# hustvl/OmniMamba

Hardware: AMD Instinct MI355X
Metric: selective-scan M-elements/sec (higher is better)
Workload: dtype bf16

## Files before the change

include/omk.h:

```cpp
#ifndef OMK_H
#define OMK_H
#include <stddef.h>
#include <stdint.h>

#ifdef __cplusplus
extern "C" {
#endif

#define OMK_ABI_VERSION 14
#define OMK_MAX_DIMS 5

typedef enum { OMK_OK = 0, OMK_EINVAL = -1, OMK_EARCH = -2, OMK_ELAUNCH = -3, OMK_EUNSUPPORTED = -4 } omk_status;
typedef enum { OMK_F32 = 0, OMK_BF16 = 1, OMK_F16 = 2, OMK_U8 = 3 , OMK_I32 = 4 ,
               OMK_F8E4M3 = 5  } omk_dtype;
typedef void* omk_stream;

typedef struct {
  void* data;
  int32_t dtype;
  int32_t ndim;
  int64_t shape[OMK_MAX_DIMS];
  int64_t stride[OMK_MAX_DIMS];
} OmkTensor;

int omk_abi_version(void);
const char* omk_last_error(void);
int omk_is_emulated(void);
size_t omk_sizeof(const char* struct_name);

typedef struct {
  OmkTensor x;
  OmkTensor residual;
// ... 55 lines not shown

typedef struct {
  OmkTensor x;
  OmkTensor weight;
  OmkTensor bias;
  OmkTensor initial_states;
  OmkTensor out;
  OmkTensor final_states;
  int32_t silu;
  OmkTensor seq_lens;
} OmkConv1dFwd;
int omk_causal_conv1d_fwd(const OmkConv1dFwd* p, omk_stream stream);

typedef struct {
  OmkTensor x, weight, bias, initial_states;
  OmkTensor dout;
  OmkTensor dx;
  OmkTensor dweight;
  OmkTensor dbias;
  OmkTensor dinitial_states;
  int32_t silu;
  void* workspace;
  size_t workspace_bytes;
} OmkConv1dBwd;
size_t omk_causal_conv1d_bwd_workspace_bytes(const OmkConv1dBwd* p);
int omk_causal_conv1d_bwd(const OmkConv1dBwd* p, omk_stream stream);

typedef struct {
  OmkTensor x;
  OmkTensor conv_state;
  OmkTensor weight, bias;
  OmkTensor out;
  int32_t silu;
  OmkTensor conv_state_indices;
  OmkTensor seq_lens;
} OmkConv1dUpdate;
int omk_causal_conv1d_update(const OmkConv1dUpdate* p, omk_stream stream);

typedef struct {
  OmkTensor state;
  OmkTensor x;
  OmkTensor dt;
  OmkTensor A;
  OmkTensor Bm, Cm;
  OmkTensor D;
  OmkTensor z;
// ... 177 lines not shown
  float top_p, temperature;
  float min_p;
} OmkSample;
int omk_sample(const OmkSample* p, omk_stream stream);

typedef struct {
  OmkTensor logits;
  OmkTensor out_ids;
  const void* top_k;
  const void* top_p;
  const void* temperature;
  const void* min_p;
  const void* seeds;
  const void* steps;
  const void* penalty;
  const void* history;
  const void* history_lens;
  const void* active;
  int64_t history_stride;
  int64_t history_cap;
} OmkSampleRows;
int omk_sample_rows(const OmkSampleRows* p, omk_stream stream);

#ifdef __cplusplus
}
#endif
#endif
```

omnimamba_amd/_capi.py:

```python
from __future__ import annotations

import ctypes as C
from typing import Optional

import torch

OMK_ABI_VERSION = 14
OMK_MAX_DIMS = 5
OMK_EUNSUPPORTED = -4
NL_FORM_GENERIC, NL_FORM_FAST, NL_FORM_BATCHED, NL_FORM_MATRIX = 0, 1, 2, 3
_DT = {torch.float32: 0, torch.bfloat16: 1, torch.float16: 2, torch.uint8: 3, torch.bool: 3, torch.int32: 4,
       torch.float8_e4m3fn: 5}


class OmkTensor(C.Structure):
    _fields_ = [("data", C.c_void_p), ("dtype", C.c_int32), ("ndim", C.c_int32),
                ("shape", C.c_int64 * OMK_MAX_DIMS), ("stride", C.c_int64 * OMK_MAX_DIMS)]


def T(t: Optional[torch.Tensor]) -> OmkTensor:
    o = OmkTensor()
    if t is None:
        return o
    dt = _DT.get(t.dtype)
    if dt is None:
        raise TypeError(f"unsupported dtype {t.dtype} (f32/bf16/f16, u8/bool masks, int32 indices, e4m3 weights only)")
    n = t.dim()
    if n > OMK_MAX_DIMS:
        raise ValueError("too many dims")
    o.data, o.dtype, o.ndim = t.data_ptr(), dt, n
# ... 1 lines not shown
    o.stride[:n] = t.stride()
    return o


def _S(name, fields):
    return type(name, (C.Structure,), {"_fields_": fields})


_t, _f, _i, _i64 = OmkTensor, C.c_float, C.c_int32, C.c_int64
_ws = [("workspace", C.c_void_p), ("workspace_bytes", C.c_size_t)]

AddNormFwd = _S("OmkAddNormFwd", [(n, _t) for n in ("x", "residual", "weight", "bias", "y", "residual_out", "rstd", "mean")]
                + [("eps", _f), ("is_rms_norm", _i)])
AddNormBwd = _S("OmkAddNormBwd", [(n, _t) for n in ("dy", "dresidual_out", "xsum", "weight", "rstd", "mean", "dx",
                                                    "dresidual_in", "dweight", "dbias")] + _ws
                + [("is_rms_norm", _i), ("has_bias", _i)])
NormGatedFwd = _S("OmkNormGatedFwd", [(n, _t) for n in ("x", "z", "weight", "bias", "y", "rstd")]
                  + [("group_size", _i64), ("eps", _f), ("norm_before_gate", _i)])
NormGatedBwd = _S("OmkNormGatedBwd", [(n, _t) for n in ("dy", "x", "z", "weight", "dx", "dz", "dweight")] + _ws
                  + [("group_size", _i64), ("eps", _f), ("norm_before_gate", _i)])
Conv1dFwd = _S("OmkConv1dFwd", [(n, _t) for n in ("x", "weight", "bias", "initial_states", "out", "final_states")]
               + [("silu", _i), ("seq_lens", _t)])
Conv1dBwd = _S("OmkConv1dBwd", [(n, _t) for n in ("x", "weight", "bias", "initial_states", "dout", "dx", "dweight",
                                                  "dbias", "dinitial_states")] + [("silu", _i), ("workspace", C.c_void_p), ("workspace_bytes", C.c_size_t)])
Conv1dUpdate = _S("OmkConv1dUpdate", [(n, _t) for n in ("x", "conv_state", "weight", "bias", "out")] + [("silu", _i), ("conv_state_indices", _t),
                                                                                                        ("seq_lens", _t)])
StateUpdate = _S("OmkStateUpdate", [(n, _t) for n in ("state", "x", "dt", "A", "Bm", "Cm", "D", "z", "dt_bias", "out")]
                 + [("dt_softplus", _i), ("state_batch_indices", _t)])
StateExtend = _S("OmkStateExtend", [(n, _t) for n in ("state", "x", "dt", "A", "Bm", "Cm", "D", "z", "dt_bias", "out")]
                 + [("dt_softplus", _i), ("state_batch_indices", _t), ("seq_lens", _t)])
SelScanFwd = _S("OmkSelScanFwd", [(n, _t) for n in ("u", "delta", "A", "Bm", "Cm", "D", "z", "delta_bias", "out",
                                                    "last_state", "pass_states")] + [("delta_softplus", _i)])
SelScanBwd = _S("OmkSelScanBwd", [(n, _t) for n in ("u", "delta", "A", "Bm", "Cm", "D", "z", "delta_bias", "dout", "du",
                                                    "ddelta", "dA", "dB", "dC", "dD", "dz", "ddelta_bias", "pass_states")] + _ws
                + [("delta_softplus", _i)])
NormLinear = _S("OmkNormLinear", [(n, _t) for n in ("x", "residual", "z", "norm_weight", "weight", "bias", "lora_a", "lora_b",
                                                    "residual_out", "out", "conv_state", "conv_weight", "conv_bias")]
                + [("group_size", C.c_int64), ("conv_offset", C.c_int64), ("eps", _f), ("lora_scale", _f),
                   ("norm_before_gate", _i), ("conv_silu", _i), ("conv_state_indices", _t),
                   ("weight_scale", _t)])
LoraAdd = _S("OmkLoraAdd", [(n, _t) for n in ("out", "h", "lora_b", "mask")] + [("scale", _f)])
LoraUpBwd = _S("OmkLoraUpBwd", [(n, _t) for n in ("dy", "lora_b", "h", "dh", "dlora_b")])
SsdFwd = _S("OmkSsdFwd", [(n, _t) for n in ("x", "dt", "A", "Bm", "Cm", "D", "z", "dt_bias", "initial_states", "out",
                                            "out_x", "final_states", "window_states")] + _ws
            + [("dt_min", _f), ("dt_max", _f), ("dt_softplus", _i), ("chunk_size", _i), ("force_generic", _i), ("flags", _i),
               ("conv_weight", _t), ("conv_bias", _t), ("seq_lens", _t)])
SSD_PRECISE, SSD_KHILO, SSD_EVERY_CHUNK, SSD_NO_SPLIT, SSD_COLUMN_SLICE, SSD_SEQUENTIAL_BWD = 1, 2, 4, 8, 16, 32
SsdBwd = _S("OmkSsdBwd", [(n, _t) for n in ("x", "dt", "A", "Bm", "Cm", "D", "dt_bias", "initial_states", "y", "dout",
                                            "dfinal_states", "dx", "ddt", "dA", "dB", "dC", "dD", "ddt_bias",
                                            "dinitial_states", "window_states")] + _ws
            + [("dt_min", _f), ("dt_max", _f), ("dt_softplus", _i), ("chunk_size", _i), ("force_generic", _i), ("flags", _i)])

CrossEntropy = _S("OmkCrossEntropy", [("logits", _t), ("labels", C.c_void_p), ("losses", _t), ("grad_scale", C.c_void_p),
                                      ("ignore_index", _i64), ("write_grad", _i)])

Sample = _S("OmkSample", [("logits", _t), ("out_ids", _t), ("step_counter", C.c_void_p), ("seed", C.c_uint64), ("offset", C.c_uint64),
                          ("top_k", _i), ("top_p", _f), ("temperature", _f), ("min_p", _f)])
SampleRows = _S("OmkSampleRows", [("logits", _t), ("out_ids", _t)]
                + [(n, C.c_void_p) for n in ("top_k", "top_p", "temperature", "min_p", "seeds", "steps", "penalty", "history", "history_lens", "active")]
                + [("history_stride", _i64), ("history_cap", _i64)])

STRUCTS = {s.__name__: s for s in (Sample, SampleRows, CrossEntropy, OmkTensor, AddNormFwd, AddNormBwd, NormGatedFwd, NormGatedBwd, Conv1dFwd, Conv1dBwd,
                                   Conv1dUpdate, StateUpdate, StateExtend, SelScanFwd, SelScanBwd, NormLinear, LoraAdd, LoraUpBwd, SsdFwd, SsdBwd)}

SYMBOLS = [
    "omk_abi_version", "omk_last_error", "omk_is_emulated", "omk_sizeof", "omk_ssd_last_kernels",
    "omk_add_norm_fwd", "omk_add_norm_bwd_workspace_bytes", "omk_add_norm_bwd",
    "omk_norm_gated_fwd", "omk_norm_gated_bwd_workspace_bytes", "omk_norm_gated_bwd",
    "omk_causal_conv1d_fwd", "omk_causal_conv1d_bwd_workspace_bytes", "omk_causal_conv1d_bwd", "omk_causal_conv1d_update",
    "omk_selective_state_update", "omk_selective_state_extend", "omk_norm_linear", "omk_norm_linear_form", "omk_lora_add", "omk_lora_up_bwd",
    "omk_selective_scan_fwd", "omk_selective_scan_fwd_form", "omk_selective_scan_bwd_form", "omk_selective_scan_bwd_workspace_bytes", "omk_selective_scan_bwd",
    "omk_ssd_scan_fwd_workspace_bytes", "omk_ssd_scan_fwd_window_states_bytes", "omk_ssd_scan_fwd", "omk_ssd_scan_bwd_workspace_bytes", "omk_ssd_scan_bwd",
    "omk_cross_entropy", "omk_lora_up_bwd_parts", "omk_sample", "omk_sample_rows",
]


def bind(lib: C.CDLL) -> C.CDLL:
    lib.omk_abi_version.restype = C.c_int
    lib.omk_last_error.restype = C.c_char_p
    lib.omk_ssd_last_kernels.restype = C.c_char_p
    lib.omk_is_emulated.restype = C.c_int
    lib.omk_sizeof.restype = C.c_size_t
    lib.omk_sizeof.argtypes = [C.c_char_p]
    for s in SYMBOLS:
        fn = getattr(lib, s)
        if s.endswith("_workspace_bytes") or s.endswith("_window_states_bytes"):
            fn.restype = C.c_size_t
            fn.argtypes = [C.c_void_p]
        elif s in ("omk_selective_scan_fwd_form", "omk_selective_scan_bwd_form", "omk_norm_linear_form"):
            fn.restype = C.c_int
            fn.argtypes = [C.c_void_p]
        elif s == "omk_lora_up_bwd_parts":
            fn.restype = C.c_int
            fn.argtypes = [C.c_int64, C.c_int64, C.POINTER(C.c_int32)]
        elif s not in ("omk_abi_version", "omk_last_error", "omk_is_emulated", "omk_sizeof", "omk_ssd_last_kernels"):
            fn.restype = C.c_int
# ... 53 lines not shown
```

omnimamba_amd/csrc/capi.hip:

```cpp
#include "omk_common.h"

namespace omk {
char* err_buf() {
  static thread_local char buf[512] = {0};
  return buf;
}
int fail(int code, const char* fmt, ...) {
  va_list ap;
  va_start(ap, fmt);
  vsnprintf(err_buf(), 512, fmt, ap);
  va_end(ap);
  return code;
}
char* kern_buf() {
  static thread_local char buf[512] = {0};
  return buf;
}
void kernels_reset() { kern_buf()[0] = 0; }
void kernels_note(const char* fmt, ...) {
  char* b = kern_buf();
  size_t n = strlen(b);
  if (n + 2 >= 512) return;
  if (n) b[n++] = ';';
  va_list ap;
// ... 2 lines not shown
  va_end(ap);
}
int finish_launch(const char* what) {
#ifndef OMK_EMU
  hipError_t e = hipGetLastError();
  if (e == hipErrorNoBinaryForGpu || e == hipErrorInvalidDeviceFunction || e == hipErrorSharedObjectInitFailed || e == hipErrorInvalidImage)
    return fail(OMK_EARCH, "%s: no kernel image for this device (%s): libomnimamba_hip is built for gfx950 (MI355X) only", what, hipGetErrorString(e));
  if (e != hipSuccess) return fail(OMK_ELAUNCH, "%s: launch failed: %s", what, hipGetErrorString(e));
#endif
  (void)what;
  return OMK_OK;
}
}

extern "C" {
int omk_abi_version(void) { return OMK_ABI_VERSION; }
const char* omk_last_error(void) { return omk::err_buf(); }
const char* omk_ssd_last_kernels(void) { return omk::kern_buf(); }
size_t omk_sizeof(const char* n) {
#define OMK_SZ(S) if (strcmp(n, #S) == 0) return sizeof(S)
  if (!n) return 0;
  OMK_SZ(OmkTensor); OMK_SZ(OmkAddNormFwd); OMK_SZ(OmkAddNormBwd); OMK_SZ(OmkNormGatedFwd); OMK_SZ(OmkNormGatedBwd);
  OMK_SZ(OmkConv1dFwd); OMK_SZ(OmkConv1dBwd); OMK_SZ(OmkConv1dUpdate); OMK_SZ(OmkStateUpdate); OMK_SZ(OmkStateExtend); OMK_SZ(OmkSelScanFwd);
  OMK_SZ(OmkSelScanBwd); OMK_SZ(OmkNormLinear); OMK_SZ(OmkLoraAdd); OMK_SZ(OmkLoraUpBwd); OMK_SZ(OmkSsdFwd); OMK_SZ(OmkSsdBwd); OMK_SZ(OmkCrossEntropy); OMK_SZ(OmkSample); OMK_SZ(OmkSampleRows);
#undef OMK_SZ
  return 0;
}
int omk_is_emulated(void) {
#ifdef OMK_EMU
  return 1;
#else
  return 0;
#endif
}
}
```

omnimamba_amd/csrc/conv1d.hip:

```cpp
#include <type_traits>
#include "omk_common.h"
#include "ssd_tiles.h"

namespace omk {

constexpr int CONV_MAXW = 4;

struct ConvArgs {
  const void* x; const void* w; const void* bias; const void* init; const void* dout;
  void* out; void* fin; void* dx; float* dw; float* db; void* dinit;
  float* part;
  int FW;
  int64_t xsb, xsc, xsl, osb, osc, osl, isb, isc, isl, fsb, fsc, fsl, dosb, dosc, dosl, dxsb, dxsc, dxsl, disb, disc, disl;
  int64_t wsc, wsk;
  int B, C, L, W, silu, wdt, bdt, idt, fdt;
  const int* lens;
};

__device__ __forceinline__ int conv_fin_end(const ConvArgs& a, int b) {
  if (!a.lens) return a.L;
  const int n = a.lens[b];
  return n < 0 ? 0 : (n > a.L ? a.L : n);
}

// ... 591 lines not shown
#pragma unroll
        for (int q = 1; q < NS; q++) v += sred[q][cvl][j];
        prow[j] = v;
      }
    }
    return;
  }
  if (strip == 0 && cvok) {
#pragma unroll
    for (int i = 0; i < VEC; i++) {
#pragma unroll
      for (int k = 0; k <= W; k++) {
        const int j = i * (W + 1) + k;
        float v = sred[0][cvl][j];
#pragma unroll
        for (int q = 1; q < NS; q++) v += sred[q][cvl][j];
        if (k < W) atomic_add_f32(a.dw + (int64_t)(c0 + i) * W + k, v);
        else if (a.db) atomic_add_f32(a.db + c0 + i, v);
      }
    }
  }
}

__global__ __launch_bounds__(1024) void conv1d_bwd_fold_kernel(const float* part, int P, int C, int W, float* dw, float* db) {
  __shared__ float sh[16][64];
  const int cl = threadIdx.x & 63, g = threadIdx.x >> 6;
  const int64_t ncol = (int64_t)C * (W + 1), col = (int64_t)blockIdx.x * 64 + cl;
  float s[4] = {0.f, 0.f, 0.f, 0.f};
  if (col < ncol) {
    for (int p0 = g; p0 < P; p0 += 64) {
      float v[4];
#pragma unroll
      for (int u = 0; u < 4; u++) { const int p = p0 + 16 * u; v[u] = p < P ? part[(int64_t)p * ncol + col] : 0.f; }
#pragma unroll
      for (int u = 0; u < 4; u++) s[u] += v[u];
    }
  }
  sh[g][cl] = (s[0] + s[1]) + (s[2] + s[3]);
  block_sync();
  if (g == 0 && col < ncol) {
    float v = 0.f;
#pragma unroll
    for (int q = 0; q < 16; q++) v += sh[q][cl];
    const int c = (int)(col / (W + 1)), k = (int)(col % (W + 1));
    if (k < W) dw[(int64_t)c * W + k] += v;
    else if (db) db[c] += v;
  }
}

template <class T>
__global__ void conv1d_bwd_generic_kernel(ConvArgs a) {
  const int64_t g = (int64_t)blockIdx.x * blockDim.x + threadIdx.x;
  if (g >= (int64_t)a.B * a.C) return;
  const int c = (int)(g % a.C), b = (int)(g / a.C), W = a.W;
  const T* x = (const T*)a.x;
  const T* dout = (const T*)a.dout;
  float w[CONV_MAXW], dwacc[CONV_MAXW] = {0.f, 0.f, 0.f, 0.f}, dbacc = 0.f;
  for (int k = 0; k < CONV_MAXW; k++) w[k] = k < W ? load_rt(a.w, (int64_t)c * a.wsc + k * a.wsk, a.wdt) : 0.f;
  const float bias = a.bias ? load_rt(a.bias, c, a.bdt) : 0.f;
  auto dpre = [&](int l) -> float {
    if (l < 0 || l >= a.L) return 0.f;
    float d = to_f32(dout[(int64_t)b * a.dosb + (int64_t)c * a.dosc + (int64_t)l * a.dosl]);
    if (a.silu) {
      float pre = bias;
      for (int k = 0; k < W; k++) pre += w[k] * conv_in<T>(a, x, b, c, l - (W - 1) + k);
      d *= silu_grad(pre);
    }
    return d;
  };
// ... 175 lines not shown
  if (!p || !present(p->x) || !present(p->weight) || !present(p->dout) || !present(p->dx) || p->x.ndim != 3 || p->weight.ndim != 2) return 0;
  if (p->x.dtype == OMK_F32) return 0;
  const int C = (int)p->x.shape[1];
  if (!(cl_fast_ok(p->x, C) && cl_fast_ok(p->dout, C) && cl_fast_ok(p->dx, C))) return 0;
  return conv_bwd_part_bytes((int)p->x.shape[0], C, (int)p->x.shape[2], (int)p->weight.shape[1]);
}

extern "C" int omk_causal_conv1d_bwd(const OmkConv1dBwd* p, omk_stream stream) {
  OMK_REQUIRE(p && present(p->x) && present(p->weight) && present(p->dout) && present(p->dx) && present(p->dweight), "causal_conv1d_bwd: x, weight, dout, dx, dweight required");
  ConvArgs a = {};
  int rc = fill_common(a, p->x, p->weight, p->bias, p->initial_states, "causal_conv1d_bwd");
  if (rc) return rc;
  OMK_REQUIRE(p->dout.dtype == p->x.dtype && p->dx.dtype == p->x.dtype, "causal_conv1d_bwd: dout/dx dtype must equal x dtype");
  OMK_REQUIRE(p->dweight.dtype == OMK_F32 && p->dweight.stride[1] == 1 && p->dweight.stride[0] == a.W, "causal_conv1d_bwd: dweight must be contiguous f32 (C, W)");
  OMK_REQUIRE(!present(p->dbias) || p->dbias.dtype == OMK_F32, "causal_conv1d_bwd: dbias must be f32");
  a.dout = p->dout.data; a.dosb = p->dout.stride[0]; a.dosc = p->dout.stride[1]; a.dosl = p->dout.stride[2];
  a.dx = p->dx.data; a.dxsb = p->dx.stride[0]; a.dxsc = p->dx.stride[1]; a.dxsl = p->dx.stride[2];
  a.dw = (float*)p->dweight.data; a.db = (float*)p->dbias.data; a.silu = p->silu;
  a.dinit = p->dinitial_states.data;
  if (present(p->dinitial_states)) {
    OMK_REQUIRE(present(p->initial_states) && p->dinitial_states.dtype == p->initial_states.dtype, "causal_conv1d_bwd: dinitial_states needs initial_states of the same dtype");
    a.disb = p->dinitial_states.stride[0]; a.disc = p->dinitial_states.stride[1]; a.disl = p->dinitial_states.stride[2];
  }
  if ((int64_t)a.B * a.C * a.L == 0) return OMK_OK;
  const bool fast = p->x.dtype != OMK_F32 && cl_fast_ok(p->x, a.C) && cl_fast_ok(p->dout, a.C) && cl_fast_ok(p->dx, a.C);
  dim3 block(256);
  if (fast) {
    constexpr int TL = 64;
#define CONV_BWD_V(T_, VEC_, TG_) do { const int CVB = (a.C / VEC_ + 63) / 64, NT4 = (a.L + 4 * TL - 1) / (4 * TL); \
      dim3 grid((unsigned)((int64_t)a.B * NT4 * CVB)); \
      if (a.W == 4) OMK_LAUNCH((conv1d_bwd_cl_kernel<T_, VEC_, TL, 4, TG_>), grid, block, 0, stream, a); \
      else if (a.W == 3) OMK_LAUNCH((conv1d_bwd_cl_kernel<T_, VEC_, TL, 3, TG_>), grid, block, 0, stream, a); \
      else OMK_LAUNCH((conv1d_bwd_cl_kernel<T_, VEC_, TL, 2, TG_>), grid, block, 0, stream, a); } while (0)
    const int64_t far = (int64_t)a.L * 2 * (a.xsl > a.dosl ? (a.xsl > a.dxsl ? a.xsl : a.dxsl) : (a.dosl > a.dxsl ? a.dosl : a.dxsl));
    if (far < ((int64_t)1 << 31) && a.xsc == 1 && a.dosc == 1 && a.dxsc == 1) {
      const bool wf = p->weight.dtype == OMK_F32 && a.wsk == 1 && a.wsc == a.W && ((uintptr_t)p->weight.data & 15) == 0 &&
                      (!present(p->bias) || (p->bias.dtype == OMK_F32 && ((uintptr_t)p->bias.data & 7) == 0));
      const int CVB = (a.C / 2 + 63) / 64, NTS = (a.L + 4 * TL - 1) / (4 * TL);
      dim3 grid((unsigned)((int64_t)a.B * NTS * CVB)), blk(256);
      const size_t pbytes = conv_bwd_part_bytes(a.B, a.C, a.L, a.W);
      a.part = (p->workspace && p->workspace_bytes >= pbytes) ? (float*)p->workspace : nullptr;
#define CONV_BWD_4G(T_, W_) do { if (wf) OMK_LAUNCH((conv1d_bwd_cl4_kernel<T_, TL, W_, TGX, 4, true>), grid, blk, 0, stream, a); \
        else OMK_LAUNCH((conv1d_bwd_cl4_kernel<T_, TL, W_, TGX, 4, false>), grid, blk, 0, stream, a); } while (0)
#define CONV_BWD_4(T_) do { if (a.W == 4) CONV_BWD_4G(T_, 4); else if (a.W == 3) CONV_BWD_4G(T_, 3); else CONV_BWD_4G(T_, 2); } while (0)
      if (p->x.dtype == OMK_BF16) CONV_BWD_4(bf16_t); else CONV_BWD_4(f16_t);
      if (a.part) {
        const int64_t ncol = (int64_t)a.C * (a.W + 1);
        OMK_LAUNCH(conv1d_bwd_fold_kernel, dim3((unsigned)((ncol + 63) / 64)), dim3(1024), 0, stream, a.part, a.B * NTS, a.C, a.W, a.dw, a.db);
      }
#undef CONV_BWD_4G
#undef CONV_BWD_4
    } else if (p->x.dtype == OMK_BF16) CONV_BWD_V(bf16_t, 2, 8); else CONV_BWD_V(f16_t, 2, 8);
#undef CONV_BWD_V
  } else {
    int64_t n = (int64_t)a.B * a.C;
    dim3 grid((unsigned)((n + 255) / 256));
    OMK_DISPATCH_DTYPE(p->x.dtype, T, OMK_LAUNCH((conv1d_bwd_generic_kernel<T>), grid, block, 0, stream, a));
  }
  if (a.dinit) {
    int64_t m = (int64_t)a.B * a.C * (a.W - 1);
    dim3 g2((unsigned)((m + 255) / 256));
    OMK_DISPATCH_DTYPE(p->x.dtype, T, OMK_LAUNCH((conv1d_dinit_kernel<T>), g2, block, 0, stream, a));
  }
  return finish_launch("causal_conv1d_bwd");
}

extern "C" int omk_causal_conv1d_update(const OmkConv1dUpdate* p, omk_stream stream) {
  OMK_REQUIRE(p && present(p->x) && present(p->conv_state) && present(p->weight) && present(p->out), "causal_conv1d_update: x, conv_state, weight, out required");
  OMK_REQUIRE(p->x.ndim == 3 && p->conv_state.ndim == 3 && p->out.ndim == 3 && p->weight.ndim == 2, "causal_conv1d_update: x/out (B, C, T), conv_state (B, C, S), weight (C, W)");
  ConvUpdArgs a = {};
  a.B = (int)p->x.shape[0]; a.C = (int)p->x.shape[1]; a.T = (int)p->x.shape[2]; a.S = (int)p->conv_state.shape[2]; a.W = (int)p->weight.shape[1];
  OMK_REQUIRE(a.W >= 2 && a.W <= CONV_MAXW && a.S >= a.W - 1, "causal_conv1d_update: W in 2..4 and state_len >= W-1");
  const bool indexed = present(p->conv_state_indices);
  OMK_REQUIRE((indexed || p->conv_state.shape[0] == a.B) && p->conv_state.shape[1] == a.C && p->weight.shape[0] == a.C, "causal_conv1d_update: shape mismatch");
  OMK_REQUIRE(indices_ok(p->conv_state_indices, a.B), "causal_conv1d_update: conv_state_indices must be contiguous int32 (B)");
  a.csi = (const int*)p->conv_state_indices.data; a.pool = (int)p->conv_state.shape[0];
  OMK_REQUIRE(indices_ok(p->seq_lens, a.B), "causal_conv1d_update: seq_lens must be contiguous int32 (B)");
// ... 16 lines not shown
```

omnimamba_amd/linear.py:

```python
from __future__ import annotations

import os

import torch
import torch.nn.functional as F

_TILE = 256


def _n_cu(device) -> int:
    try:
        return torch.cuda.get_device_properties(device).multi_processor_count
    except Exception:
        return 256


def split_factor(m: int, n: int, k: int, device) -> int:
    if os.environ.get("OMK_WGRAD_SPLITK", "1") == "0":
        return 1
    cu = _n_cu(device)
    tiles = -(-m // _TILE) * -(-n // _TILE)

    def eff(s):
        items = s * tiles
        return items / (-(-items // cu) * cu)

    if eff(1) >= 0.75:
        return 1
    best = 1
    cands, kmin = ((2, 4, 8, 16, 32), 512) if tiles <= 16 else ((2, 4, 8), 2048)
    for s in cands:
        if k % s or k // s < kmin:
            break
        best = s
        if eff(s) >= 0.8:
            break
    return best


def weight_grad(dy2d: torch.Tensor, x2d: torch.Tensor, out_dtype: torch.dtype) -> torch.Tensor:
    k, m = dy2d.shape
    n = x2d.shape[1]
    if (dy2d.is_cuda and dy2d.dtype in (torch.bfloat16, torch.float16) and dy2d.is_contiguous() and x2d.is_contiguous()):
        s = split_factor(m, n, k, dy2d.device)
        if s > 1:
            part = torch.bmm(dy2d.view(s, k // s, m).transpose(1, 2), x2d.view(s, k // s, n), out_dtype=torch.float32)
            return part.sum(0).to(out_dtype)
    return (dy2d.t() @ x2d).to(out_dtype)


class _XGradFn(torch.autograd.Function):

    @staticmethod
    @torch.amp.custom_fwd(device_type="cuda")
    def forward(ctx, x, weight, bias):
        if torch.is_autocast_enabled():
            adt = torch.get_autocast_dtype("cuda")
            x, weight = x.to(adt), weight.to(adt)
            bias = None if bias is None else bias.to(adt)
        ctx.save_for_backward(weight)
        return F.linear(x, weight, bias)

    @staticmethod
    @torch.amp.custom_bwd(device_type="cuda")
    def backward(ctx, dy):
        (weight,) = ctx.saved_tensors
        return (dy @ weight.to(dy.dtype)) if ctx.needs_input_grad[0] else None, None, None


class _WGradFn(torch.autograd.Function):
# ... 51 lines not shown
```

omnimamba_amd/ssd_combined.py:

```python
from __future__ import annotations

import math
import os

import torch
import torch.nn.functional as F

from . import _capi as K
from . import _prof
from ._lib import forward_only_seq_lens, get_lib, require_device, slot_indices
from .causal_conv1d import causal_conv1d_fn
from .layernorm_gated import rmsnorm_fn
from .linear import frozen_cast, weight_grad

_INF = float("inf")


def _last_contig(t):
    return t if t is None or t.stride(-1) == 1 else t.contiguous()


import contextlib
import threading

# ... 101 lines not shown
                     out=K.T(bc.transpose(1, 2)), final_states=K.T(None if conv_state_out is None else conv_state_out[:, d_ssm:]), silu=1,
                     seq_lens=K.T(seq_lens))
    K.run(lib, "omk_causal_conv1d_fwd", pc, xBC)
    with _prof.range_("ssd_scan_fwd_fused_conv"):
        if not K.try_run(lib, "omk_ssd_scan_fwd", p, xBC):
            return None
    if conv_state_out is not None:
        sl = conv_state_out.shape[-1]
        cs = conv_state_out[:, :d_ssm]
        if seq_lens is not None:
            pos = seq_lens.long()[:, None] + torch.arange(-sl, 0, device=xBC.device)
            rows = xBC[:, :, :d_ssm].gather(1, pos.clamp(0, L - 1)[..., None].expand(-1, -1, d_ssm))
            cs.copy_(rows.masked_fill_((pos < 0)[..., None], 0).transpose(1, 2))
        elif L >= sl:
            cs.copy_(xBC[:, L - sl:, :d_ssm].transpose(1, 2))
        else:
            cs[..., :sl - L].zero_()
            cs[..., sl - L:].copy_(xBC[:, :, :d_ssm].transpose(1, 2))
    return out, fin


def ssd_scan_bwd(dout, x, dt, A, B, C, D=None, dt_bias=None, initial_states=None, dfinal_states=None,
                 dt_softplus=False, dt_limit=(0.0, _INF), chunk_size=256, need_dinit=False, force_generic=False, y=None,
                 dx_out=None, dB_out=None, dC_out=None, window_states=None, flags=None):
    lib = get_lib()
    x, B, C, dout, y = _last_contig(x), _last_contig(B), _last_contig(C), _last_contig(dout), _last_contig(y)
    if y is not None and y.dtype != x.dtype:
        y = y.to(x.dtype)
    if B.dtype != x.dtype:
        B = B.to(x.dtype)
    if C.dtype != x.dtype:
        C = C.to(x.dtype)
    if dout.dtype != x.dtype:
        dout = dout.to(x.dtype)
    A = A.float().contiguous()
    Bsz, L, H, P = x.shape
    G, N = B.shape[2], B.shape[3]
    dev = x.device
    dx = dx_out if dx_out is not None else torch.empty(Bsz, L, H, P, dtype=x.dtype, device=dev)
    ddt = torch.empty(Bsz, H, L, dtype=torch.float32, device=dev).transpose(1, 2)
    dA = torch.empty(H, dtype=torch.float32, device=dev)
    dB = dB_out if dB_out is not None else torch.empty(Bsz, L, G, N, dtype=x.dtype, device=dev)
    dC = dC_out if dC_out is not None else torch.empty(Bsz, L, G, N, dtype=x.dtype, device=dev)
    dD = None if D is None else torch.empty(D.shape, dtype=torch.float32, device=dev)
    ddtb = None if dt_bias is None else torch.empty(H, dtype=torch.float32, device=dev)
    dinit = torch.empty(Bsz, H, P, N, dtype=torch.float32, device=dev) if need_dinit else None
    if dfinal_states is not None:
        dfinal_states = dfinal_states.float()
    if x.numel() > 0:
        p = K.SsdBwd(x=K.T(x), dt=K.T(dt), A=K.T(A), Bm=K.T(B), Cm=K.T(C), D=K.T(D), dt_bias=K.T(dt_bias),
                     initial_states=K.T(initial_states), y=K.T(y), dout=K.T(dout), dfinal_states=K.T(dfinal_states), dx=K.T(dx),
                     ddt=K.T(ddt), dA=K.T(dA), dB=K.T(dB), dC=K.T(dC), dD=K.T(dD), ddt_bias=K.T(ddtb),
                     dinitial_states=K.T(dinit), window_states=K.T(window_states), dt_min=float(dt_limit[0]), dt_max=float(dt_limit[1]),
                     dt_softplus=int(dt_softplus), chunk_size=int(chunk_size), force_generic=int(force_generic),
                     flags=int(current_scan_flags() if flags is None else flags) & (K.SSD_EVERY_CHUNK | K.SSD_NO_SPLIT | K.SSD_COLUMN_SLICE | K.SSD_SEQUENTIAL_BWD))
        ws = K.workspace(lib, "omk_ssd_scan_bwd_workspace_bytes", p, x)
        with _prof.range_("ssd_scan_bwd"):
            K.run(lib, "omk_ssd_scan_bwd", p, x)
        _prof.note_kernels("ssd_scan_bwd", lib)
    else:
        for t in (dA, dD, ddtb):
            if t is not None:
                t.zero_()
# ... 207 lines not shown
        if outproj_w is not None:
            w_c = getattr(ctx, "w_cast", None)
            d_outn = dout @ (w_c if (w_c is not None and w_c.dtype == adt) else outproj_w.to(adt))
            if need_wo:
                do2, on2 = dout.reshape(-1, dout.shape[-1]), on.reshape(-1, d_ssm)
                d_outproj_w = weight_grad(do2 if do2.is_contiguous() else do2.contiguous(), on2 if on2.is_contiguous() else on2.contiguous(),
                                          outproj_w.dtype)
            if outproj_b is not None and ctx.needs_input_grad[15]:
                d_outproj_b = dout.reshape(-1, dout.shape[-1]).sum(0).to(outproj_b.dtype)
        else:
            d_outn = dout
        d_norm_w = None
        if use_norm:
            rows = Bsz * L
            y_r = y2.reshape(rows, d_ssm)
            z_r = z.as_strided((rows, d_ssm), (zxbcdt.stride(1), 1), z.storage_offset()) if zxbcdt.stride(0) == L * zxbcdt.stride(1) else z.reshape(rows, d_ssm)
            dz_r = dz.as_strided((rows, d_ssm), (dzxbcdt.stride(1), 1), dz.storage_offset())
            g_r = d_outn.reshape(rows, d_ssm)
            if g_r.dtype != adt:
                g_r = g_r.to(adt)
            if g_r.stride(-1) != 1:
                g_r = g_r.contiguous()
            dy = torch.empty(Bsz, L, d_ssm, dtype=adt, device=dev)
            gw = torch.zeros(d_ssm, dtype=torch.float32, device=dev) if ctx.needs_input_grad[12] else None
            pn = K.NormGatedBwd(dy=K.T(g_r), x=K.T(y_r), z=K.T(z_r), weight=K.T(norm_w), dx=K.T(dy.reshape(rows, d_ssm)),
                                dz=K.T(dz_r), dweight=K.T(gw), group_size=d_ssm // G, eps=eps, norm_before_gate=int(nbg))
            wsn = K.workspace(lib, "omk_norm_gated_bwd_workspace_bytes", pn, g_r)
            K.run(lib, "omk_norm_gated_bwd", pn, g_r)
            d_norm_w = None if gw is None else gw.to(norm_w.dtype)
        else:
            zf = z.float()
            dz.copy_((d_outn.float() * y2.float() * _silu_grad(zf)).to(adt))
            dy = (d_outn.float() * F.silu(zf)).to(adt)
        if xBC_saved is not None:
            xBC_c = xBC_saved
        else:
            with torch.no_grad():
                xBC_c = causal_conv1d_fn(xBC.transpose(1, 2), conv_w, conv_b, activation=activation).transpose(1, 2)
        x, Bm, Cm = torch.split(xBC_c, [d_ssm, G * N, G * N], dim=-1)
        dxBC_c = torch.empty_like(xBC_c)
        dx_v, dB_v, dC_v = torch.split(dxBC_c, [d_ssm, G * N, G * N], dim=-1)
        g = ssd_scan_bwd(dy.reshape(Bsz, L, H, P), x.unflatten(-1, (H, P)), dt, A, Bm.unflatten(-1, (G, N)),
                         Cm.unflatten(-1, (G, N)), D=D, dt_bias=dt_bias, initial_states=initial_states,
                         dfinal_states=dfinal, dt_softplus=True, dt_limit=dt_limit, chunk_size=chunk_size,
                         need_dinit=initial_states is not None, y=y_pre, dx_out=dx_v.unflatten(-1, (H, P)),
                         dB_out=dB_v.unflatten(-1, (G, N)), dC_out=dC_v.unflatten(-1, (G, N)), window_states=wst,
                         flags=ctx.scan_flags)
        ddt_v.copy_(g["ddt"])
        dw = torch.zeros(conv_w.shape, dtype=torch.float32, device=dev)
        db = None if conv_b is None else torch.zeros(conv_b.shape, dtype=torch.float32, device=dev)
        p = K.Conv1dBwd(x=K.T(xBC.transpose(1, 2)), weight=K.T(conv_w), bias=K.T(conv_b), initial_states=K.T(None),
                        dout=K.T(dxBC_c.transpose(1, 2)), dx=K.T(dxBC.transpose(1, 2)), dweight=K.T(dw), dbias=K.T(db),
                        dinitial_states=K.T(None), silu=1)
        cws = K.workspace(lib, "omk_causal_conv1d_bwd_workspace_bytes", p, zxbcdt)
        K.run(lib, "omk_causal_conv1d_bwd", p, zxbcdt)
        dinit = g["dinitial_states"]
        return (dzxbcdt, dw.to(conv_w.dtype), None if conv_b is None else db.to(conv_b.dtype),
                g["ddt_bias"].to(dt_bias.dtype), g["dA"].to(A.dtype), g["dD"].to(D.dtype), None,
                None if dinit is None else dinit.to(initial_states.dtype), None, None, None, None, d_norm_w, None,
                d_outproj_w, d_outproj_b, None, None, None, None, None)


def mamba_split_conv1d_scan_combined(zxbcdt, conv1d_weight, conv1d_bias, dt_bias, A, D, chunk_size, initial_states=None,
                                     seq_idx=None, dt_limit=(0.0, _INF), return_final_states=False, activation="silu",
                                     rmsnorm_weight=None, rmsnorm_eps=1e-6, outproj_weight=None, outproj_bias=None,
                                     headdim=None, ngroups=1, norm_before_gate=True, conv_state_out=None, seq_lens=None):
    forward_only_seq_lens(seq_lens, zxbcdt, conv1d_weight, conv1d_bias, dt_bias, A, D, initial_states, rmsnorm_weight, outproj_weight, outproj_bias)
    return MambaSplitConv1dScanCombinedFn.apply(zxbcdt, conv1d_weight, conv1d_bias, dt_bias, A, D, chunk_size,
                                                initial_states, seq_idx, dt_limit, return_final_states, activation,
                                                rmsnorm_weight, rmsnorm_eps, outproj_weight, outproj_bias, headdim,
                                                ngroups, norm_before_gate, conv_state_out, seq_lens)
```

Before: 23660.

## Add fused split-K fold kernel and skip zero-fills in backward gradients

Adds a fold_partials kernel that sums split-K f32 partials and writes the result in the output dtype, replacing torch sum plus cast. Adds a plan for weight-grad GEMMs that computes whole rounds of tiles directly and applies split-K only to the remainder. Lets conv1d backward and the gated-norm backward write their weight gradients by assignment, so the zero-fill launches can be dropped. Also threads a ddt_out parameter through. These all sit on training backward paths, not on the selective-scan forward that is measured.

```diff
diff --git a/include/omk.h b/include/omk.h
--- a/include/omk.h
+++ b/include/omk.h
@@ -7,7 +7,7 @@
 extern "C" {
 #endif
 
-#define OMK_ABI_VERSION 14
+#define OMK_ABI_VERSION 15
 #define OMK_MAX_DIMS 5
 
 typedef enum { OMK_OK = 0, OMK_EINVAL = -1, OMK_EARCH = -2, OMK_ELAUNCH = -3, OMK_EUNSUPPORTED = -4 } omk_status;
@@ -109,6 +109,7 @@
   int32_t silu;
   void* workspace;
   size_t workspace_bytes;
+  int32_t outputs_uninit;
 } OmkConv1dBwd;
 size_t omk_causal_conv1d_bwd_workspace_bytes(const OmkConv1dBwd* p);
 int omk_causal_conv1d_bwd(const OmkConv1dBwd* p, omk_stream stream);
@@ -332,6 +333,12 @@
 } OmkSampleRows;
 int omk_sample_rows(const OmkSampleRows* p, omk_stream stream);
 
+typedef struct {
+  OmkTensor part;
+  OmkTensor out;
+} OmkFoldPartials;
+int omk_fold_partials(const OmkFoldPartials* p, omk_stream stream);
+
 #ifdef __cplusplus
 }
 #endif
diff --git a/omnimamba_amd/_capi.py b/omnimamba_amd/_capi.py
--- a/omnimamba_amd/_capi.py
+++ b/omnimamba_amd/_capi.py
@@ -5,7 +5,7 @@
 
 import torch
 
-OMK_ABI_VERSION = 14
+OMK_ABI_VERSION = 15
 OMK_MAX_DIMS = 5
 OMK_EUNSUPPORTED = -4
 NL_FORM_GENERIC, NL_FORM_FAST, NL_FORM_BATCHED, NL_FORM_MATRIX = 0, 1, 2, 3
@@ -53,7 +53,8 @@
 Conv1dFwd = _S("OmkConv1dFwd", [(n, _t) for n in ("x", "weight", "bias", "initial_states", "out", "final_states")]
                + [("silu", _i), ("seq_lens", _t)])
 Conv1dBwd = _S("OmkConv1dBwd", [(n, _t) for n in ("x", "weight", "bias", "initial_states", "dout", "dx", "dweight",
-                                                  "dbias", "dinitial_states")] + [("silu", _i), ("workspace", C.c_void_p), ("workspace_bytes", C.c_size_t)])
+                                                  "dbias", "dinitial_states")] + [("silu", _i), ("workspace", C.c_void_p), ("workspace_bytes", C.c_size_t),
+                                                                                ("outputs_uninit", _i)])
 Conv1dUpdate = _S("OmkConv1dUpdate", [(n, _t) for n in ("x", "conv_state", "weight", "bias", "out")] + [("silu", _i), ("conv_state_indices", _t),
                                                                                                         ("seq_lens", _t)])
 StateUpdate = _S("OmkStateUpdate", [(n, _t) for n in ("state", "x", "dt", "A", "Bm", "Cm", "D", "z", "dt_bias", "out")]
@@ -90,8 +91,9 @@
 SampleRows = _S("OmkSampleRows", [("logits", _t), ("out_ids", _t)]
                 + [(n, C.c_void_p) for n in ("top_k", "top_p", "temperature", "min_p", "seeds", "steps", "penalty", "history", "history_lens", "active")]
                 + [("history_stride", _i64), ("history_cap", _i64)])
+FoldPartials = _S("OmkFoldPartials", [("part", _t), ("out", _t)])
 
-STRUCTS = {s.__name__: s for s in (Sample, SampleRows, CrossEntropy, OmkTensor, AddNormFwd, AddNormBwd, NormGatedFwd, NormGatedBwd, Conv1dFwd, Conv1dBwd,
+STRUCTS = {s.__name__: s for s in (FoldPartials, Sample, SampleRows, CrossEntropy, OmkTensor, AddNormFwd, AddNormBwd, NormGatedFwd, NormGatedBwd, Conv1dFwd, Conv1dBwd,
                                    Conv1dUpdate, StateUpdate, StateExtend, SelScanFwd, SelScanBwd, NormLinear, LoraAdd, LoraUpBwd, SsdFwd, SsdBwd)}
 
 SYMBOLS = [
@@ -102,7 +104,7 @@
     "omk_selective_state_update", "omk_selective_state_extend", "omk_norm_linear", "omk_norm_linear_form", "omk_lora_add", "omk_lora_up_bwd",
     "omk_selective_scan_fwd", "omk_selective_scan_fwd_form", "omk_selective_scan_bwd_form", "omk_selective_scan_bwd_workspace_bytes", "omk_selective_scan_bwd",
     "omk_ssd_scan_fwd_workspace_bytes", "omk_ssd_scan_fwd_window_states_bytes", "omk_ssd_scan_fwd", "omk_ssd_scan_bwd_workspace_bytes", "omk_ssd_scan_bwd",
-    "omk_cross_entropy", "omk_lora_up_bwd_parts", "omk_sample", "omk_sample_rows",
+    "omk_cross_entropy", "omk_lora_up_bwd_parts", "omk_sample", "omk_sample_rows", "omk_fold_partials",
 ]
 
 
diff --git a/omnimamba_amd/csrc/capi.hip b/omnimamba_amd/csrc/capi.hip
--- a/omnimamba_amd/csrc/capi.hip
+++ b/omnimamba_amd/csrc/capi.hip
@@ -48,7 +48,7 @@
   if (!n) return 0;
   OMK_SZ(OmkTensor); OMK_SZ(OmkAddNormFwd); OMK_SZ(OmkAddNormBwd); OMK_SZ(OmkNormGatedFwd); OMK_SZ(OmkNormGatedBwd);
   OMK_SZ(OmkConv1dFwd); OMK_SZ(OmkConv1dBwd); OMK_SZ(OmkConv1dUpdate); OMK_SZ(OmkStateUpdate); OMK_SZ(OmkStateExtend); OMK_SZ(OmkSelScanFwd);
-  OMK_SZ(OmkSelScanBwd); OMK_SZ(OmkNormLinear); OMK_SZ(OmkLoraAdd); OMK_SZ(OmkLoraUpBwd); OMK_SZ(OmkSsdFwd); OMK_SZ(OmkSsdBwd); OMK_SZ(OmkCrossEntropy); OMK_SZ(OmkSample); OMK_SZ(OmkSampleRows);
+  OMK_SZ(OmkSelScanBwd); OMK_SZ(OmkNormLinear); OMK_SZ(OmkLoraAdd); OMK_SZ(OmkLoraUpBwd); OMK_SZ(OmkSsdFwd); OMK_SZ(OmkSsdBwd); OMK_SZ(OmkCrossEntropy); OMK_SZ(OmkSample); OMK_SZ(OmkSampleRows); OMK_SZ(OmkFoldPartials);
 #undef OMK_SZ
   return 0;
 }
diff --git a/omnimamba_amd/csrc/conv1d.hip b/omnimamba_amd/csrc/conv1d.hip
--- a/omnimamba_amd/csrc/conv1d.hip
+++ b/omnimamba_amd/csrc/conv1d.hip
@@ -637,7 +637,7 @@
   }
 }
 
-__global__ __launch_bounds__(1024) void conv1d_bwd_fold_kernel(const float* part, int P, int C, int W, float* dw, float* db) {
+__global__ __launch_bounds__(1024) void conv1d_bwd_fold_kernel(const float* part, int P, int C, int W, float* dw, float* db, int assign) {
   __shared__ float sh[16][64];
   const int cl = threadIdx.x & 63, g = threadIdx.x >> 6;
   const int64_t ncol = (int64_t)C * (W + 1), col = (int64_t)blockIdx.x * 64 + cl;
@@ -658,8 +658,8 @@
 #pragma unroll
     for (int q = 0; q < 16; q++) v += sh[q][cl];
     const int c = (int)(col / (W + 1)), k = (int)(col % (W + 1));
-    if (k < W) dw[(int64_t)c * W + k] += v;
-    else if (db) db[c] += v;
+    if (k < W) dw[(int64_t)c * W + k] = (assign ? 0.f : dw[(int64_t)c * W + k]) + v;
+    else if (db) db[c] = (assign ? 0.f : db[c]) + v;
   }
 }
 
@@ -881,7 +881,8 @@
     OMK_REQUIRE(present(p->initial_states) && p->dinitial_states.dtype == p->initial_states.dtype, "causal_conv1d_bwd: dinitial_states needs initial_states of the same dtype");
     a.disb = p->dinitial_states.stride[0]; a.disc = p->dinitial_states.stride[1]; a.disl = p->dinitial_states.stride[2];
   }
-  if ((int64_t)a.B * a.C * a.L == 0) return OMK_OK;
+  static const char* const uninit_msg = "causal_conv1d_bwd: outputs_uninit needs the workspace path (16-bit channel-last views + workspace): zero dweight / dbias and pass 0";
+  if ((int64_t)a.B * a.C * a.L == 0) return p->outputs_uninit ? fail(OMK_EUNSUPPORTED, uninit_msg) : OMK_OK;
   const bool fast = p->x.dtype != OMK_F32 && cl_fast_ok(p->x, a.C) && cl_fast_ok(p->dout, a.C) && cl_fast_ok(p->dx, a.C);
   dim3 block(256);
   if (fast) {
@@ -899,19 +900,22 @@
       dim3 grid((unsigned)((int64_t)a.B * NTS * CVB)), blk(256);
       const size_t pbytes = conv_bwd_part_bytes(a.B, a.C, a.L, a.W);
       a.part = (p->workspace && p->workspace_bytes >= pbytes) ? (float*)p->workspace : nullptr;
+      if (p->outputs_uninit && !a.part) return fail(OMK_EUNSUPPORTED, uninit_msg);
 #define CONV_BWD_4G(T_, W_) do { if (wf) OMK_LAUNCH((conv1d_bwd_cl4_kernel<T_, TL, W_, TGX, 4, true>), grid, blk, 0, stream, a); \
         else OMK_LAUNCH((conv1d_bwd_cl4_kernel<T_, TL, W_, TGX, 4, false>), grid, blk, 0, stream, a); } while (0)
 #define CONV_BWD_4(T_) do { if (a.W == 4) CONV_BWD_4G(T_, 4); else if (a.W == 3) CONV_BWD_4G(T_, 3); else CONV_BWD_4G(T_, 2); } while (0)
       if (p->x.dtype == OMK_BF16) CONV_BWD_4(bf16_t); else CONV_BWD_4(f16_t);
       if (a.part) {
         const int64_t ncol = (int64_t)a.C * (a.W + 1);
-        OMK_LAUNCH(conv1d_bwd_fold_kernel, dim3((unsigned)((ncol + 63) / 64)), dim3(1024), 0, stream, a.part, a.B * NTS, a.C, a.W, a.dw, a.db);
+        OMK_LAUNCH(conv1d_bwd_fold_kernel, dim3((unsigned)((ncol + 63) / 64)), dim3(1024), 0, stream, a.part, a.B * NTS, a.C, a.W, a.dw, a.db, p->outputs_uninit ? 1 : 0);
       }
 #undef CONV_BWD_4G
 #undef CONV_BWD_4
-    } else if (p->x.dtype == OMK_BF16) CONV_BWD_V(bf16_t, 2, 8); else CONV_BWD_V(f16_t, 2, 8);
+    } else if (p->outputs_uninit) return fail(OMK_EUNSUPPORTED, uninit_msg);
+    else if (p->x.dtype == OMK_BF16) CONV_BWD_V(bf16_t, 2, 8); else CONV_BWD_V(f16_t, 2, 8);
 #undef CONV_BWD_V
   } else {
+    if (p->outputs_uninit) return fail(OMK_EUNSUPPORTED, uninit_msg);
     int64_t n = (int64_t)a.B * a.C;
     dim3 grid((unsigned)((n + 255) / 256));
     OMK_DISPATCH_DTYPE(p->x.dtype, T, OMK_LAUNCH((conv1d_bwd_generic_kernel<T>), grid, block, 0, stream, a));
diff --git a/omnimamba_amd/csrc/fold.hip b/omnimamba_amd/csrc/fold.hip
--- /dev/null
+++ b/omnimamba_amd/csrc/fold.hip
@@ -0,0 +1,100 @@
+#include "omk_common.h"
+
+namespace omk {
+
+struct FoldArgs {
+  const float* part; void* out;
+  int64_t n;
+  int64_t cols, ld;
+  int S, odt, strided;
+};
+
+__device__ __forceinline__ int64_t fold_out_offset(const FoldArgs& a, int64_t i) {
+  if (!a.strided) return i;
+  const int64_t r = i / a.cols;
+  return r * a.ld + (i - r * a.cols);
+}
+
+template <class TO, int SMAX, bool EXACT, int U>
+__global__ __launch_bounds__(256) void fold_vec_kernel(FoldArgs a) {
+  const int64_t nvec = a.n >> 2;
+  const int nt = (int)blockDim.x;
+  const int64_t v0 = (int64_t)blockIdx.x * (nt * U) + threadIdx.x;
+  const int S = EXACT ? SMAX : a.S;
+  f32x4 r[U][SMAX];
+#pragma unroll
+  for (int u = 0; u < U; u++) {
+    int64_t v = v0 + u * nt;
+    if (v >= nvec) v = nvec - 1;
+    const float* src = a.part + (v << 2);
+#pragma unroll
+    for (int s = 0; s < SMAX; s++)
+      if (EXACT || s < S) r[u][s] = *reinterpret_cast<const f32x4*>(src + (int64_t)s * a.n);
+  }
+#pragma unroll
+  for (int u = 0; u < U; u++) {
+    const int64_t v = v0 + u * nt;
+    f32x4 acc = r[u][0];
+#pragma unroll
+    for (int s = 1; s < SMAX; s++)
+      if (EXACT || s < S) acc += r[u][s];
+    if (v < nvec) {
+      const float o[4] = {acc[0], acc[1], acc[2], acc[3]};
+      store_vec<TO, 4>((TO*)a.out + fold_out_offset(a, v << 2), o);
+    }
+  }
+}
+
+__global__ __launch_bounds__(256) void fold_scalar_kernel(FoldArgs a) {
+  const int64_t i = (int64_t)blockIdx.x * 256 + threadIdx.x;
+  if (i >= a.n) return;
+  float acc = a.part[i];
+  for (int s = 1; s < a.S; s++) acc += a.part[(int64_t)s * a.n + i];
+  store_rt(a.out, fold_out_offset(a, i), a.odt, acc);
+}
+
+}
+
+using namespace omk;
+
+extern "C" int omk_fold_partials(const OmkFoldPartials* p, omk_stream stream) {
+  OMK_REQUIRE(p && present(p->part) && present(p->out), "fold_partials: part, out required");
+  OMK_REQUIRE(p->part.dtype == OMK_F32 && (p->part.ndim == 2 || p->part.ndim == 3) && is_dense(p->part), "fold_partials: part must be dense f32 (S, n) or (S, rows, cols)");
+  OMK_REQUIRE(p->out.ndim == p->part.ndim - 1, "fold_partials: out must have the shape of one slice");
+  OMK_REQUIRE(p->out.dtype == OMK_F32 || p->out.dtype == OMK_BF16 || p->out.dtype == OMK_F16, "fold_partials: out must be f32, bf16 or f16");
+  FoldArgs a = {};
+  a.S = (int)p->part.shape[0];
+  OMK_REQUIRE(p->part.shape[0] >= 2 && p->part.shape[0] <= 32, "fold_partials: 2 .. 32 slices, got %lld", (long long)p->part.shape[0]);
+  for (int i = 0; i < p->out.ndim; i++) OMK_REQUIRE(p->out.shape[i] == p->part.shape[i + 1], "fold_partials: out / part shape mismatch");
+  a.n = numel(p->out);
+  if (a.n == 0) return OMK_OK;
+  a.cols = p->out.shape[p->out.ndim - 1];
+  OMK_REQUIRE(a.cols == 1 || p->out.stride[p->out.ndim - 1] == 1, "fold_partials: out needs unit stride on its last dimension");
+  a.ld = p->out.ndim == 2 ? p->out.stride[0] : a.cols;
+  if (p->out.ndim == 2 && p->out.shape[0] > 1) OMK_REQUIRE(a.ld >= a.cols, "fold_partials: rows of out overlap");
+  a.strided = (p->out.ndim == 2 && p->out.shape[0] > 1 && a.ld != a.cols) ? 1 : 0;
+  a.part = (const float*)p->part.data; a.out = p->out.data; a.odt = p->out.dtype;
+  {
+    const uintptr_t p0 = (uintptr_t)a.part, p1 = p0 + (size_t)a.S * a.n * 4;
+    const int64_t last = a.strided ? (p->out.shape[0] - 1) * a.ld + a.cols : a.n;
+    const uintptr_t o0 = (uintptr_t)a.out, o1 = o0 + (size_t)last * dtype_size(a.odt);
+    OMK_REQUIRE(o1 <= p0 || o0 >= p1, "fold_partials: out overlaps part");
+  }
+  const size_t osz = dtype_size(a.odt);
+  const bool vec = a.n % 4 == 0 && aligned16(p->part) && ((uintptr_t)a.out % (4 * osz)) == 0 && (!a.strided || (a.cols % 4 == 0 && a.ld % 4 == 0));
+  if (!vec) {
+    OMK_LAUNCH(fold_scalar_kernel, dim3((unsigned)((a.n + 255) / 256)), dim3(256), 0, stream, a);
+    return finish_launch("fold_partials");
+  }
+  const int64_t nvec = a.n / 4;
+#define FOLD_GO(TO, SMAX, EXACT, U) do { const int nt = nvec < (int64_t)2048 * 256 * U ? 64 : 256; \
+  OMK_LAUNCH((fold_vec_kernel<TO, SMAX, EXACT, U>), dim3((unsigned)((nvec + nt * U - 1) / (nt * U))), dim3(nt), 0, stream, a); } while (0)
+#define FOLD_S(TO) do { \
+    if (a.S == 2) FOLD_GO(TO, 2, true, 2); else if (a.S == 3) FOLD_GO(TO, 3, true, 2); else if (a.S == 4) FOLD_GO(TO, 4, true, 2); \
+    else if (a.S == 8) FOLD_GO(TO, 8, true, 1); else if (a.S == 16) FOLD_GO(TO, 16, true, 1); else if (a.S == 32) FOLD_GO(TO, 32, true, 1); \
+    else if (a.S < 8) FOLD_GO(TO, 8, false, 1); else if (a.S < 16) FOLD_GO(TO, 16, false, 1); else FOLD_GO(TO, 32, false, 1); } while (0)
+  OMK_DISPATCH_DTYPE(a.odt, TO, FOLD_S(TO));
+#undef FOLD_S
+#undef FOLD_GO
+  return finish_launch("fold_partials");
+}
diff --git a/omnimamba_amd/linear.py b/omnimamba_amd/linear.py
--- a/omnimamba_amd/linear.py
+++ b/omnimamba_amd/linear.py
@@ -15,10 +15,7 @@
         return 256
 
 
-def split_factor(m: int, n: int, k: int, device) -> int:
-    if os.environ.get("OMK_WGRAD_SPLITK", "1") == "0":
-        return 1
-    cu = _n_cu(device)
+def _split(m: int, n: int, k: int, cu: int) -> int:
     tiles = -(-m // _TILE) * -(-n // _TILE)
 
     def eff(s):
@@ -38,14 +35,63 @@
     return best
 
 
+def split_factor(m: int, n: int, k: int, device) -> int:
+    if os.environ.get("OMK_WGRAD_SPLITK", "1") == "0":
+        return 1
+    return _split(m, n, k, _n_cu(device))
+
+
+def weight_grad_plan(m: int, n: int, k: int, cu: int):
+    if os.environ.get("OMK_WGRAD_SPLITK", "1") == "0":
+        return 0, 1
+    s_all = _split(m, n, k, cu)
+    tiles_n = -(-n // _TILE)
+    tiles = -(-m // _TILE) * tiles_n
+    if tiles / (-(-tiles // cu) * cu) >= 0.9 or cu % tiles_n or n % _TILE or (m, n, k) in _NO_EXACT_ROUND:
+        return 0, s_all
+    r = cu // tiles_n
+    rounds = (m // _TILE) // r
+    m_main = rounds * r * _TILE
+    rest = m - m_main
+    if rounds == 0 or rest == 0 or -(-rest // _TILE) * tiles_n >= 0.75 * cu:
+        return 0, s_all
+    return m_main, _split(rest, n, k, cu)
+
+
+_NO_EXACT_ROUND = frozenset()
+
+
+def fold_partials(part: torch.Tensor, out: torch.Tensor) -> torch.Tensor:
+    from . import _capi as K
+    from ._lib import get_lib, require_device
+    lib = get_lib()
+    require_device(lib, part, out)
+    K.run(lib, "omk_fold_partials", K.FoldPartials(part=K.T(part), out=K.T(out)), part)
+    return out
+
+
+def _split_gemm(dy2d, x2d, s, out):
+    k, m = dy2d.shape
+    n = x2d.shape[1]
+    part = torch.bmm(dy2d.unflatten(0, (s, k // s)).transpose(1, 2), x2d.view(s, k // s, n), out_dtype=torch.float32)
+    return fold_partials(part, out)
+
+
 def weight_grad(dy2d: torch.Tensor, x2d: torch.Tensor, out_dtype: torch.dtype) -> torch.Tensor:
     k, m = dy2d.shape
     n = x2d.shape[1]
     if (dy2d.is_cuda and dy2d.dtype in (torch.bfloat16, torch.float16) and dy2d.is_contiguous() and x2d.is_contiguous()):
-        s = split_factor(m, n, k, dy2d.device)
+        m_main, s = weight_grad_plan(m, n, k, _n_cu(dy2d.device))
+        if m_main:
+            dw = torch.empty(m, n, dtype=torch.float32, device=dy2d.device)
+            torch.mm(dy2d[:, :m_main].t(), x2d, out_dtype=torch.float32, out=dw[:m_main])
+            if s > 1:
+                _split_gemm(dy2d[:, m_main:], x2d, s, dw[m_main:])
+            else:
+                torch.mm(dy2d[:, m_main:].t(), x2d, out_dtype=torch.float32, out=dw[m_main:])
+            return dw.to(out_dtype)
         if s > 1:
-            part = torch.bmm(dy2d.view(s, k // s, m).transpose(1, 2), x2d.view(s, k // s, n), out_dtype=torch.float32)
-            return part.sum(0).to(out_dtype)
+            return _split_gemm(dy2d, x2d, s, torch.empty(m, n, dtype=out_dtype, device=dy2d.device))
     return (dy2d.t() @ x2d).to(out_dtype)
 
 
diff --git a/omnimamba_amd/ssd_combined.py b/omnimamba_amd/ssd_combined.py
--- a/omnimamba_amd/ssd_combined.py
+++ b/omnimamba_amd/ssd_combined.py
@@ -147,7 +147,7 @@
 
 def ssd_scan_bwd(dout, x, dt, A, B, C, D=None, dt_bias=None, initial_states=None, dfinal_states=None,
                  dt_softplus=False, dt_limit=(0.0, _INF), chunk_size=256, need_dinit=False, force_generic=False, y=None,
-                 dx_out=None, dB_out=None, dC_out=None, window_states=None, flags=None):
+                 dx_out=None, dB_out=None, dC_out=None, window_states=None, flags=None, ddt_out=None):
     lib = get_lib()
     x, B, C, dout, y = _last_contig(x), _last_contig(B), _last_contig(C), _last_contig(dout), _last_contig(y)
     if y is not None and y.dtype != x.dtype:
@@ -163,7 +163,7 @@
     G, N = B.shape[2], B.shape[3]
     dev = x.device
     dx = dx_out if dx_out is not None else torch.empty(Bsz, L, H, P, dtype=x.dtype, device=dev)
-    ddt = torch.empty(Bsz, H, L, dtype=torch.float32, device=dev).transpose(1, 2)
+    ddt = ddt_out if ddt_out is not None else torch.empty(Bsz, H, L, dtype=torch.float32, device=dev).transpose(1, 2)
     dA = torch.empty(H, dtype=torch.float32, device=dev)
     dB = dB_out if dB_out is not None else torch.empty(Bsz, L, G, N, dtype=x.dtype, device=dev)
     dC = dC_out if dC_out is not None else torch.empty(Bsz, L, G, N, dtype=x.dtype, device=dev)
@@ -417,7 +417,7 @@
             if g_r.stride(-1) != 1:
                 g_r = g_r.contiguous()
             dy = torch.empty(Bsz, L, d_ssm, dtype=adt, device=dev)
-            gw = torch.zeros(d_ssm, dtype=torch.float32, device=dev) if ctx.needs_input_grad[12] else None
+            gw = (torch.empty if rows else torch.zeros)(d_ssm, dtype=torch.float32, device=dev) if ctx.needs_input_grad[12] else None
             pn = K.NormGatedBwd(dy=K.T(g_r), x=K.T(y_r), z=K.T(z_r), weight=K.T(norm_w), dx=K.T(dy.reshape(rows, d_ssm)),
                                 dz=K.T(dz_r), dweight=K.T(gw), group_size=d_ssm // G, eps=eps, norm_before_gate=int(nbg))
             wsn = K.workspace(lib, "omk_norm_gated_bwd_workspace_bytes", pn, g_r)
@@ -442,13 +442,18 @@
                          dB_out=dB_v.unflatten(-1, (G, N)), dC_out=dC_v.unflatten(-1, (G, N)), window_states=wst,
                          flags=ctx.scan_flags)
         ddt_v.copy_(g["ddt"])
-        dw = torch.zeros(conv_w.shape, dtype=torch.float32, device=dev)
-        db = None if conv_b is None else torch.zeros(conv_b.shape, dtype=torch.float32, device=dev)
+        dw = torch.empty(conv_w.shape, dtype=torch.float32, device=dev)
+        db = None if conv_b is None else torch.empty(conv_b.shape, dtype=torch.float32, device=dev)
         p = K.Conv1dBwd(x=K.T(xBC.transpose(1, 2)), weight=K.T(conv_w), bias=K.T(conv_b), initial_states=K.T(None),
                         dout=K.T(dxBC_c.transpose(1, 2)), dx=K.T(dxBC.transpose(1, 2)), dweight=K.T(dw), dbias=K.T(db),
-                        dinitial_states=K.T(None), silu=1)
+                        dinitial_states=K.T(None), silu=1, outputs_uninit=1)
         cws = K.workspace(lib, "omk_causal_conv1d_bwd_workspace_bytes", p, zxbcdt)
-        K.run(lib, "omk_causal_conv1d_bwd", p, zxbcdt)
+        if not K.try_run(lib, "omk_causal_conv1d_bwd", p, zxbcdt):
+            dw.zero_()
+            if db is not None:
+                db.zero_()
+            p.outputs_uninit = 0
+            K.run(lib, "omk_causal_conv1d_bwd", p, zxbcdt)
         dinit = g["dinitial_states"]
         return (dzxbcdt, dw.to(conv_w.dtype), None if conv_b is None else db.to(conv_b.dtype),
                 g["ddt_bias"].to(dt_bias.dtype), g["dA"].to(A.dtype), g["dD"].to(D.dtype), None,
```

Result: faster. 24360 (median of 6 runs) (+3.0%).
